# hieunghia-pat/OpenViIC

Measured on AMD Instinct MI355X. Metric: captions/sec (whole node) at beam=5, 50 regions x d2048, higher is better.
Workload: dtype f32; 1 GPU; standard_transformer beam=5, B=256 per GPU, 50x2048 synthetic regions, V=10201, max_len=20, random-init weights; global_batch=256, parallelism=dp1, streams=4

## Files before the change

### include/ovc.h

```cpp
#ifndef OVC_H_
#define OVC_H_

#include <stddef.h>
#include <stdint.h>

#ifdef __cplusplus
extern "C" {
#endif

typedef void* ovc_stream;

#define OVC_OK            0
#define OVC_EINVAL       -1
#define OVC_EWORKSPACE   -2
#define OVC_ELAUNCH      -3
#define OVC_EDEVICE      -4

#define OVC_MAX_LAYERS    8
#define OVC_MAX_LEVELS    4
#define OVC_MAX_BEAM      8
#define OVC_MAX_SEGMENTS  8
#define OVC_MAX_REGIONS   1024
#define OVC_MAX_LEN       256

// ... 302 lines not shown

int ovc_debug_force_gemm_tiling(int tiling);
int ovc_debug_clear_tuning(void);
int ovc_debug_linear_tiling(const float* x, int K, const float* W, const float* bias, float* y, int M, int N,
                            int tiling, int ksplit, int iters, ovc_stream stream);
int ovc_debug_attention_mem_backward(const float* q, const float* k, const float* v, const float* dout, const uint8_t* mask,
                                     const float* m_k, const float* m_v, int B, int n, int h, int dk, int m, float* P, float* dS,
                                     float* dq, float* dk_out, float* dv_out, float* part_k, float* part_v, float* colpart,
                                     float* d_mk, float* d_mv, ovc_stream stream);

size_t ovc_debug_vocab_select_bytes(int B, int width, int V, int k);
int ovc_debug_vocab_select(const float* x, const float* fc, const float* running, const float* alive, int B, int width,
                           int V, int d, int k, int transposed, int kchains, void* scratch, size_t scratch_bytes, int64_t* chosen,
                           float* score, ovc_stream stream);

size_t ovc_split_weight_bytes(int N, int K, int mode);
int ovc_split_weight(const float* W, int N, int K, int mode, void* planes, ovc_stream stream);
int ovc_debug_linear_planes(const float* x, int K, const float* W, const void* planes, const float* bias, float* y,
                            int M, int N, int tiling, int ksplit, int iters, ovc_stream stream);
int ovc_debug_repeat_linear(const float* x, int K, const float* W, const float* bias, float* y,
                            int M, int N, int iters, ovc_stream stream);

size_t ovc_debug_decode_self_partial_bytes(int t, int rows, int h, int d_k);
int ovc_debug_decode_self_attention(const float* q, int ldq, const float* kcache, const float* vcache, size_t pos_stride, int ldkv,
                                    const int32_t* anc, int anc_ld, const uint8_t* padflag, int pad_ld, int t, int width, int rows,
                                    int h, int d_k, float* out, int ldo, void* partials, size_t partial_bytes, const int32_t* gate,
                                    int per_row, ovc_stream stream);
int ovc_debug_decode_cross_attention(const float* q, int ldq, const float* kx, const float* vx, size_t level_stride, int ldkv,
                                     const uint8_t* encmask, int N, int width, int B, int heads, int d_k, int levels, float* out,
                                     size_t out_level_stride, int ldo, const int32_t* gate, ovc_stream stream);
int ovc_debug_decode_self_form(int t, int width, int rows, int h, int d_k, int per_row);
int ovc_debug_decode_cross_form(int N, int width, int h, int d_k);

typedef struct {
    const float* teacher_logp;
    float weight;
} ovc_distill;
size_t ovc_train_distill_workspace_bytes(const ovc_model* m, int B, int N, int T, int dropout);
int ovc_forward_backward_distill(const ovc_model* m, const ovc_model* grads, const float* features, const float* boxes, int B, int N,
                                 const int64_t* tokens, const int64_t* targets, int T, void* workspace, size_t workspace_bytes,
                                 float* loss_out, int use_graph, ovc_stream stream, const ovc_distill* distill,
                                 const ovc_dropout* dropout);
int ovc_ensemble_combine(const float* const* logps, int M, long rows, int V, int renormalise, float* out, ovc_stream stream);

#ifdef __cplusplus
}
#endif
#endif
```

### openviic_amd/csrc/attention.hip

```cpp
#include <cstdlib>
#include <mutex>

#include "common.h"

namespace {

constexpr int kQTile = 64;
constexpr int kLdQK = 68;

struct AttnArgs {
    const float* q; const float* k; const float* v; float* out;
    int b, nq, nk, h, dk, dv;
    const uint8_t* mask; long mask_sb, mask_sq;
    const float* geometry;
    const float* mem_k; const float* mem_v; int m; float mem_scale_k, mem_scale_v;
    int nkp;
    int qtiles;
};

__global__ __launch_bounds__(256) void attention_mfma_kernel(AttnArgs p) {
    extern __shared__ __attribute__((aligned(16))) float lds[];
    const int tid = threadIdx.x, lane = tid & 63, wave = tid >> 6;
    const int qt = blockIdx.x % p.qtiles;
    const int hd = (blockIdx.x / p.qtiles) % p.h;
// ... 474 lines not shown
                                      hipFuncAttributeMaxDynamicSharedMemorySize, 96 * 1024);                         \
        });                                                                                                           \
        hipLaunchKernelGGL((attention_tiled_kernel<KG, DVT>), grid, block, bytes, ovc_hip_stream(stream), p);         \
    } while (0)
        if (hmax <= 16) OVC_ATT_TILED(2, 1); else if (hmax <= 32) OVC_ATT_TILED(4, 1); else OVC_ATT_TILED(8, 2);
#undef OVC_ATT_TILED
        OVC_RETURN_IF_LAUNCH_FAILED();
        return OVC_OK;
    }
    const size_t lds_bytes = sizeof(float) * ((size_t)kQTile * kLdQK + 2 * (size_t)p.nkp * kLdQK + (size_t)kQTile * (p.nkp + 4));
    static std::once_flag attr_once;
    std::call_once(attr_once, [] {
        (void)hipFuncSetAttribute(reinterpret_cast<const void*>(attention_mfma_kernel),
                                  hipFuncAttributeMaxDynamicSharedMemorySize, 128 * 1024);
    });
    hipLaunchKernelGGL(attention_mfma_kernel, dim3(b * h * p.qtiles), dim3(256), lds_bytes, ovc_hip_stream(stream), p);
    OVC_RETURN_IF_LAUNCH_FAILED();
    return OVC_OK;
}


constexpr int kSelfMaxHeads = 32;

template <int CH, int KB = 1>
__global__ __launch_bounds__(256) void decode_self_attention_kernel(DecodeSelfArgs p) {
#include "bodies/decode_self_attention_kernel.inc"
}
template <int CH, int KB = 1>
__global__ __launch_bounds__(256) void decode_self_attention_kernel_gated(DecodeSelfArgs p, const int32_t* __restrict__ gate) {
    if (ovc_gate_closed(gate)) return;
#include "bodies/decode_self_attention_kernel.inc"
}

template <int NT, int SB, bool CHUNKED = false>
__global__ __launch_bounds__(256) void decode_self_attention_mfma_kernel(DecodeSelfArgs p) {
#include "bodies/decode_self_attention_mfma_kernel.inc"
}
template <int NT, int SB, bool CHUNKED = false>
__global__ __launch_bounds__(256) void decode_self_attention_mfma_kernel_gated(DecodeSelfArgs p, const int32_t* __restrict__ gate) {
    if (ovc_gate_closed(gate)) return;
#include "bodies/decode_self_attention_mfma_kernel.inc"
}

__global__ __launch_bounds__(256) void decode_self_merge_kernel(DecodeSelfArgs p, int rows, int chunks) {
#include "bodies/decode_self_merge_kernel.inc"
}
__global__ __launch_bounds__(256) void decode_self_merge_kernel_gated(DecodeSelfArgs p, int rows, int chunks, const int32_t* __restrict__ gate) {
    if (ovc_gate_closed(gate)) return;
#include "bodies/decode_self_merge_kernel.inc"
}

constexpr int kFormSelfMfma = 100, kFormSelfChunked = 200, kFormSelfRows = 300;
constexpr int kFormCrossMfma = 400, kFormCrossTiled = 500, kFormCrossLds = 600;

static int decode_self_form(int t, int W, int rows, int h, int dk, bool per_row) {
    if (t < 0 || t >= OVC_MAX_LEN || h <= 0 || h > kSelfMaxHeads) return OVC_EINVAL;
    if ((dk & (dk - 1)) || dk < 4 || dk > 64) return OVC_EINVAL;
    const int hk = h * dk;
    if (hk > 1024) return OVC_EINVAL;
    const bool per_image = !per_row && W >= 1 && W <= OVC_MAX_BEAM && rows % W == 0 && dk >= 16;
    const int SB = dk >> 4, CH = hk <= 256 ? 1 : hk <= 512 ? 2 : 4;
    if (t >= 64) {
        if (per_image) return kFormSelfChunked + (W <= 1 ? 1 : W <= 2 ? 2 : W <= 4 ? 4 : W <= 5 ? 5 : 8) * 10 + SB;
        return kFormSelfRows + CH * 10 + 4;
    }
    const int worst = t == 0 ? 1 : W * (t + 1);
    if (per_image && worst <= 112) {
        const int tiles = (worst + 15) / 16;
        return kFormSelfMfma + (tiles <= 1 ? 1 : tiles <= 2 ? 2 : tiles <= 4 ? 4 : 7) * 10 + SB;
    }
    return kFormSelfRows + CH * 10 + 1;
}

static int decode_self_attention_as(const DecodeSelfArgs& p, int rows, bool per_row, hipStream_t stream, const int32_t* gate) {
    if (p.dk != p.dv) return OVC_EINVAL;
    const int form = decode_self_form(p.t, p.width, rows, p.h, p.dk, per_row);
    if (form < 0) return form;
    const int W = p.width;
    const bool chunked = form >= kFormSelfChunked && form < kFormSelfRows;
    if (chunked && (!p.part_o || !p.part_ml)) return OVC_EINVAL;
    const int chunks = (p.t + kSelfChunk) / kSelfChunk;
    switch (form) {
#define OVC_SELF(NT, SB)                                                                                             \
    case kFormSelfMfma + NT * 10 + SB: {                                                                             \
        const dim3 grid(rows / W, (p.h + 3) / 4), block(256);                                                        \
        if (gate) hipLaunchKernelGGL((decode_self_attention_mfma_kernel_gated<NT, SB>), grid, block, 0, stream, p, gate); \
        else hipLaunchKernelGGL((decode_self_attention_mfma_kernel<NT, SB>), grid, block, 0, stream, p);            \
    } break
#define OVC_SELF_CHUNKED(NT, SB)                                                                                     \
    case kFormSelfChunked + NT * 10 + SB: {                                                                          \
        const dim3 grid(rows / W, (p.h + 3) / 4, chunks), block(256);                                                \
        if (gate) hipLaunchKernelGGL((decode_self_attention_mfma_kernel_gated<NT, SB, true>), grid, block, 0, stream, p, gate); \
        else hipLaunchKernelGGL((decode_self_attention_mfma_kernel<NT, SB, true>), grid, block, 0, stream, p);      \
    } break
#define OVC_SELF_ROWS(CH, KB)                                                                                        \
    case kFormSelfRows + CH * 10 + KB:                                                                               \
        if (gate) hipLaunchKernelGGL((decode_self_attention_kernel_gated<CH, KB>), dim3(rows), dim3(256), 0, stream, p, gate); \
        else hipLaunchKernelGGL((decode_self_attention_kernel<CH, KB>), dim3(rows), dim3(256), 0, stream, p);       \
        break
#define OVC_SELF_SB(M, NT) M(NT, 1); M(NT, 2); M(NT, 4)
        OVC_SELF_SB(OVC_SELF, 1); OVC_SELF_SB(OVC_SELF, 2); OVC_SELF_SB(OVC_SELF, 4); OVC_SELF_SB(OVC_SELF, 7);
        OVC_SELF_SB(OVC_SELF_CHUNKED, 1); OVC_SELF_SB(OVC_SELF_CHUNKED, 2); OVC_SELF_SB(OVC_SELF_CHUNKED, 4);
        OVC_SELF_SB(OVC_SELF_CHUNKED, 5); OVC_SELF_SB(OVC_SELF_CHUNKED, 8);
        OVC_SELF_ROWS(1, 1); OVC_SELF_ROWS(2, 1); OVC_SELF_ROWS(4, 1);
        OVC_SELF_ROWS(1, 4); OVC_SELF_ROWS(2, 4); OVC_SELF_ROWS(4, 4);
#undef OVC_SELF_SB
#undef OVC_SELF_ROWS
#undef OVC_SELF_CHUNKED
#undef OVC_SELF
        default: return OVC_EINVAL;
    }
    OVC_RETURN_IF_LAUNCH_FAILED();
    if (chunked) {
// ... 112 lines not shown

extern "C" size_t ovc_debug_decode_self_partial_bytes(int t, int rows, int h, int d_k) {
    if (t < 64 || t >= OVC_MAX_LEN || rows < 1 || !debug_heads_ok(h, d_k)) return 0;
    const size_t chunks = (size_t)(t + kSelfChunk) / kSelfChunk;
    return sizeof(float) * chunks * rows * ((size_t)h * d_k + 2 * (size_t)h);
}

extern "C" int ovc_debug_decode_self_attention(const float* q, int ldq, const float* kcache, const float* vcache, size_t pos_stride,
                                               int ldkv, const int32_t* anc, int anc_ld, const uint8_t* padflag, int pad_ld, int t,
                                               int width, int rows, int h, int d_k, float* out, int ldo, void* partials,
                                               size_t partial_bytes, const int32_t* gate, int per_row, ovc_stream stream) {
    if (!q || !kcache || !vcache || !padflag || !out || (t > 0 && !anc)) return OVC_EINVAL;
    if (!debug_self_shape_ok(t, width, rows, h, d_k)) return OVC_EINVAL;
    const int hk = h * d_k;
    if (ldq < hk || ldkv < hk || ldo < hk || (ldq & 3) || (ldkv & 3) || (ldo & 3) || (pos_stride & 3)) return OVC_EINVAL;
    if (anc_ld < t || pad_ld < rows) return OVC_EINVAL;
    if (!ovc_aligned16(q) || !ovc_aligned16(kcache) || !ovc_aligned16(vcache) || !ovc_aligned16(out)) return OVC_EINVAL;
    const size_t need = ovc_debug_decode_self_partial_bytes(t, rows, h, d_k);
    if (need && (!partials || !ovc_aligned16(partials) || partial_bytes < need)) return OVC_EINVAL;
    if (const int rc = ovc_device_guard()) return rc;
    DecodeSelfArgs p{};
    p.q = q; p.ldq = ldq; p.kcache = kcache; p.vcache = vcache; p.pos_stride = pos_stride; p.ldkv = ldkv;
    p.anc = anc; p.anc_ld = anc_ld; p.padflag = padflag; p.pad_ld = pad_ld;
    p.t = t; p.width = width; p.h = h; p.dk = d_k; p.dv = d_k;
    p.out = out; p.ldo = ldo;
    if (need) {
        const size_t chunks = (size_t)(t + kSelfChunk) / kSelfChunk;
        p.part_o = static_cast<float*>(partials);
        p.part_ml = p.part_o + chunks * rows * hk;
    }
    return decode_self_attention_as(p, rows, per_row != 0, ovc_hip_stream(stream), gate);
}

extern "C" int ovc_debug_decode_cross_attention(const float* q, int ldq, const float* kx, const float* vx, size_t level_stride, int ldkv,
                                                const uint8_t* encmask, int N, int width, int B, int heads, int d_k, int levels,
                                                float* out, size_t out_level_stride, int ldo, const int32_t* gate, ovc_stream stream) {
    if (!q || !kx || !vx || !out || B < 1 || levels < 1 || levels > OVC_MAX_LEVELS) return OVC_EINVAL;
    if (!debug_cross_shape_ok(N, width, heads, d_k)) return OVC_EINVAL;
    const int hk = heads * d_k;
    if (ldq < hk || ldkv < hk || ldo < hk || (ldq & 3) || (ldkv & 3) || (ldo & 3) || (level_stride & 3) || (out_level_stride & 3)) return OVC_EINVAL;
    if (!ovc_aligned16(q) || !ovc_aligned16(kx) || !ovc_aligned16(vx) || !ovc_aligned16(out)) return OVC_EINVAL;
    if (const int rc = ovc_device_guard()) return rc;
    DecodeCrossArgs p{};
    p.q = q; p.ldq = ldq; p.kx = kx; p.vx = vx; p.level_stride = level_stride; p.ldkv = ldkv;
    p.encmask = encmask; p.n = N; p.width = width; p.heads = heads; p.dk = d_k; p.dv = d_k;
    p.out = out; p.out_level_stride = out_level_stride; p.ldo = ldo;
    return ovc_decode_cross_attention(p, B, heads, levels, ovc_hip_stream(stream), gate);
}
```

### openviic_amd/csrc/bodies/decode_self_attention_mfma_kernel.inc

```
    constexpr int kPos = CHUNKED ? kSelfChunk : 64;
    __shared__ unsigned short keyinfo[NT * 16];
    __shared__ uint8_t keypad[NT * 16];
    __shared__ uint8_t sl[OVC_MAX_BEAM][kPos];
    __shared__ int nkeys_shared;
    const int lane = threadIdx.x & 63, wave = threadIdx.x >> 6;
    const int b = blockIdx.x, t = p.t, W = p.width;
    const int j0 = CHUNKED ? (int)blockIdx.z * kSelfChunk : 0;
    const int hd = min((int)blockIdx.y * 4 + wave, p.h - 1);
    const bool live = (int)blockIdx.y * 4 + wave < p.h;
    const int r = lane & 15, kq = lane >> 4;

    const float* qg = p.q + (size_t)(b * W + min(r, W - 1)) * p.ldq + hd * p.dk;
    f32x4 qf[SB];
#pragma unroll
    for (int S = 0; S < SB; ++S) qf[S] = *reinterpret_cast<const f32x4*>(qg + 16 * S + 4 * kq);

    if (wave == 0) {
        const int j = j0 + lane;
        const int wj = j == 0 ? 1 : W;
        int slot[OVC_MAX_BEAM];
        uint8_t pad[OVC_MAX_BEAM];
        unsigned mask = 0;
        if (j <= t && lane < kPos) {
#pragma unroll
            for (int i = 0; i < OVC_MAX_BEAM; ++i)
                slot[i] = i < W ? (j == t ? i : p.anc[(size_t)(b * W + i) * p.anc_ld + j] - b * wj) : 0;
#pragma unroll
            for (int l = 0; l < OVC_MAX_BEAM; ++l) pad[l] = l < wj ? p.padflag[(size_t)j * p.pad_ld + b * wj + l] : 0;
#pragma unroll
            for (int i = 0; i < OVC_MAX_BEAM; ++i)
                if (i < W) {
                    const int s = min(max(slot[i], 0), wj - 1);
                    sl[i][j - j0] = (uint8_t)s;
                    mask |= 1u << s;
                }
        }
        const int cnt = __popc(mask);
        int incl = cnt;
#pragma unroll
        for (int off = 1; off < 64; off <<= 1) {
            const int up = __shfl_up(incl, off, 64);
            if (lane >= off) incl += up;
        }
        int n = incl - cnt;
#pragma unroll
        for (int l = 0; l < OVC_MAX_BEAM; ++l)
            if (mask & (1u << l)) {
                if (n < NT * 16) { keyinfo[n] = (unsigned short)((j << 3) | l); keypad[n] = pad[l]; }
                ++n;
            }
        if (lane == 63) nkeys_shared = min(incl, NT * 16);
    }
    __syncthreads();
    const int nkeys = nkeys_shared;

    f32x4 kf[NT][SB];
#pragma unroll
    for (int T = 0; T < NT; ++T) {
        if (16 * T < nkeys) {
            const int info = keyinfo[min(16 * T + r, nkeys - 1)];
            const int j = info >> 3, l = info & 7;
            const float* krow = p.kcache + (size_t)j * p.pos_stride + (size_t)(b * (j == 0 ? 1 : W) + l) * p.ldkv + hd * p.dk + 4 * kq;
#pragma unroll
            for (int S = 0; S < SB; ++S) kf[T][S] = *reinterpret_cast<const f32x4*>(krow + 16 * S);
        }
    }
    if (r >= W) {
#pragma unroll
        for (int S = 0; S < SB; ++S) qf[S] = f32x4{0.f, 0.f, 0.f, 0.f};
    }
    f32x4 st[NT];
#pragma unroll
    for (int T = 0; T < NT; ++T) st[T] = f32x4{0.f, 0.f, 0.f, 0.f};
#pragma unroll
    for (int T = 0; T < NT; ++T) {
        if (16 * T < nkeys) {
#pragma unroll
            for (int S = 0; S < SB; ++S)
#pragma unroll
                for (int e = 0; e < 4; ++e) st[T] = __builtin_amdgcn_mfma_f32_16x16x4f32(kf[T][S][e], qf[S][e], st[T], 0, 0, 0);
        }
    }

    const int vc = 4 * min(r, (p.dv >> 2) - 1);
    f32x4 vf[NT][4];
#pragma unroll
    for (int T = 0; T < NT; ++T) {
        if (16 * T < nkeys) {
#pragma unroll
            for (int g = 0; g < 4; ++g) {
                const int info = keyinfo[min(16 * T + 4 * kq + g, nkeys - 1)];
                const int j = info >> 3, l = info & 7;
                vf[T][g] = *reinterpret_cast<const f32x4*>(p.vcache + (size_t)j * p.pos_stride +
                                                           (size_t)(b * (j == 0 ? 1 : W) + l) * p.ldkv + hd * p.dv + vc);
            }
        }
    }

    const float scale_div = sqrtf((float)p.dk);
    const int beam = min(r, W - 1);
    float mx = -INFINITY;
#pragma unroll
    for (int T = 0; T < NT; ++T) {
#pragma unroll
        for (int g = 0; g < 4; ++g) {
            const int key = 16 * T + 4 * kq + g;
            float s = -INFINITY;
            if (key < nkeys) {
                const int info = keyinfo[key];
                if (!keypad[key] && sl[beam][(info >> 3) - j0] == (info & 7)) s = st[T][g] / scale_div;
            }
            st[T][g] = s;
            mx = fmaxf(mx, s);
        }
    }
    mx = fmaxf(mx, __shfl_xor(mx, 16, 64));
    mx = fmaxf(mx, __shfl_xor(mx, 32, 64));
    const float mref = CHUNKED && mx == -INFINITY ? 0.f : mx;
    float sum = 0.f;
#pragma unroll
    for (int T = 0; T < NT; ++T)
#pragma unroll
        for (int g = 0; g < 4; ++g) {
            const float e = expf(st[T][g] - mref);
            st[T][g] = e;
            sum += e;
        }
    sum += __shfl_xor(sum, 16, 64);
    sum += __shfl_xor(sum, 32, 64);
    if constexpr (!CHUNKED) {
#pragma unroll
        for (int T = 0; T < NT; ++T)
#pragma unroll
            for (int g = 0; g < 4; ++g) st[T][g] = st[T][g] / sum;
    }

    f32x4 acc[4];
#pragma unroll
    for (int e = 0; e < 4; ++e) acc[e] = f32x4{0.f, 0.f, 0.f, 0.f};
#pragma unroll
    for (int T = 0; T < NT; ++T) {
        if (16 * T < nkeys) {
#pragma unroll
            for (int g = 0; g < 4; ++g)
#pragma unroll
                for (int e = 0; e < 4; ++e) acc[e] = __builtin_amdgcn_mfma_f32_16x16x4f32(vf[T][g][e], st[T][g], acc[e], 0, 0, 0);
        }
    }
    if (live && r < W) {
        float* orow;
        if constexpr (CHUNKED) {
            const size_t prow = (size_t)blockIdx.z * gridDim.x * W + b * W + r;
            orow = p.part_o + prow * p.h * p.dv + hd * p.dv;
            if (kq == 0) reinterpret_cast<float2*>(p.part_ml)[prow * p.h + hd] = make_float2(mx, sum);
        } else {
            orow = p.out + (size_t)(b * W + r) * p.ldo + hd * p.dv;
        }
#pragma unroll
        for (int g = 0; g < 4; ++g) {
            const int dvb = 16 * kq + 4 * g;
            if (dvb < p.dv) *reinterpret_cast<f32x4*>(orow + dvb) = f32x4{acc[0][g], acc[1][g], acc[2][g], acc[3][g]};
        }
    }
```

### openviic_amd/csrc/common.h

```cpp
#pragma once
#include <hip/hip_runtime.h>
#include <stdint.h>
#include "../../include/ovc.h"

#define OVC_WAVE 64

#define OVC_RETURN_IF_LAUNCH_FAILED()                      \
    do {                                                   \
        if (hipGetLastError() != hipSuccess) return OVC_ELAUNCH; \
    } while (0)

typedef float f32x2 __attribute__((ext_vector_type(2)));
typedef float f32x4 __attribute__((ext_vector_type(4)));
typedef float f32x16 __attribute__((ext_vector_type(16)));

static inline hipStream_t ovc_hip_stream(ovc_stream s) { return reinterpret_cast<hipStream_t>(s); }

int ovc_device_guard();

static inline bool ovc_aligned16(const void* p) { return (reinterpret_cast<uintptr_t>(p) & 15u) == 0; }

#ifdef OVC_MEASUREMENT_HOOKS
#include <cstdlib>
#define OVC_HOOK_ENV(name) getenv(name)
// ... 102 lines not shown
    int drop_cols = 0;
};

int ovc_gemm_launch(const GemmArgs& args, hipStream_t stream, const GemmLaunchOpts& opts = GemmLaunchOpts{});
int ovc_gemm_pick_tiling(const GemmArgs& args, const GemmLaunchOpts& opts = GemmLaunchOpts{});
int ovc_gemm_tiling_class(int tiling);
constexpr int kMaxKSplit = 4;
int ovc_layer_norm_parts(const float* parts, int nparts, long part_stride, const float* bias, const float* residual,
                         const float* gamma, const float* beta, const uint8_t* zero_rows, float eps, float* y,
                         int rows, int d, hipStream_t stream, const int32_t* gate = nullptr);
int ovc_layer_norm_gated(const float* x, const float* residual, const float* gamma, const float* beta, const float* add, int add_rows,
                         const uint8_t* zero_rows, float eps, float* y, int rows, int d, hipStream_t stream, const int32_t* gate);
int ovc_sigmoid_gate_gated(const float* a, const float* g, float* y, long n, hipStream_t stream, const int32_t* gate);
const char* ovc_gemm_tiling_name(int tiling);

struct DecodeSelfArgs {
    const float* q;
    int ldq;
    const float* kcache;
    const float* vcache;
    size_t pos_stride;
    int ldkv;
    const int32_t* anc;
    int anc_ld;
    const uint8_t* padflag;
    int pad_ld;
    int t;
    int width;
    int h, dk, dv;
    float* out;
    int ldo;
    float* part_o;
    float* part_ml;
};
constexpr int kSelfChunk = 16;
int ovc_decode_self_attention(const DecodeSelfArgs& p, int rows, hipStream_t stream, const int32_t* gate = nullptr);

struct DecodeCrossArgs {
    const float* q;
    int ldq;
    const float* kx;
    const float* vx;
    size_t level_stride;
    int ldkv;
    const uint8_t* encmask;
    int n, width;
    int heads, dk, dv;
    float* out;
    size_t out_level_stride;
    int ldo;
};
int ovc_decode_cross_attention(const DecodeCrossArgs& p, int B, int h, int levels, hipStream_t stream, const int32_t* gate = nullptr);

struct BeamSelectArgs {
    const float* logits;
    int ld;
    int is_logp;
    const float* running;
    const float* alive;
    int width, V, k;
    float* cand_v;
    int* cand_i;
    int64_t* chosen;
    float* score;
    float* masked_logp;
    float* row_max_out;
    float* row_lsum_out;
// ... 99 lines not shown
```

### openviic_amd/csrc/engine.hip

```cpp
#include <algorithm>
#include <array>
#include <cstdlib>
#include <list>
#include <map>
#include <memory>
#include <atomic>
#include <cmath>
#include <mutex>
#include <tuple>
#include <vector>

#include "common.h"
#include "backward.h"
#include "dropout.h"

namespace {

#define TRY(expr)                          \
    do {                                   \
        const int _rc = (expr);            \
        if (_rc != OVC_OK) return _rc;     \
    } while (0)
#define RUN(expr)                          \
    do {                                   \
// ... 38 lines not shown
        }
        (void)hipEventDestroy(r.start); (void)hipEventDestroy(r.stop);
    }
    g_profile.clear();
}

struct Bump {
    char* base; size_t off;
    template <typename T> T* take(size_t count) {
        off = (off + 255) & ~(size_t)255;
        T* p = base ? reinterpret_cast<T*>(base + off) : nullptr;
        off += count * sizeof(T);
        return p;
    }
};

struct EncTape { float *q, *k, *v, *att, *ya, *x1, *ff, *yf, *out; };
struct DecTape { float *q, *k, *v, *att, *ys, *x1, *qc, *attc, *yc, *x2, *ff, *yf, *out; };
struct ClTape { float *k[2], *v[2], *att, *ya, *o2p, *a1, *h2; };
struct Tape { EncTape enc[OVC_MAX_LAYERS]; DecTape dec[OVC_MAX_LAYERS]; ClTape cl; };

struct Workspace {
    const Tape* tape;
    uint8_t* enc_mask; float* pe; float* xe[2]; float* eq; float* ek; float* ev; float* eatt; float* ey;
    float* eff; float* einfo; float* egate; float* geometry; float* enc_levels;
    float* kx; float* vx;
    float* cl_out; float* cl_cat; float* cl_q;
    float* x; float* x1; float* x2; float* y; float* q; float* att; float* ff; float* info; float* gate;
    float* enc_att; float* alpha; float* mixed; float* ymesh;
    float* part;
    float* kc; float* vc;
    uint8_t* padflag;
    float* sa_part_o; float* sa_part_ml;
    float* logits;
    float* stats;
    float* running[2]; float* alive[2]; int32_t* hist[2]; float* lp[2]; int32_t* anc[2];
    int32_t* tok; float* cand_v; int32_t* cand_i; float* row_max; float* row_lsum; int32_t* order;
    float* all_buf;
    int64_t* out_ids; float* out_logp;
    int32_t* alive_count;
    int64_t* drop_seed; int32_t* steps_dev;
    float* choice_rows; int32_t* choice_word; int32_t* choice_kept;
    uint8_t* self_mask; int32_t* tgt; float* tgt_logit; float* lse;
    Workspace* peers;
    size_t bytes;
};

int enc_heads(const ovc_model* m) { return m->enc_heads ? m->enc_heads : m->heads; }
int enc_dk(const ovc_model* m) { return m->enc_d_k ? m->enc_d_k : m->d_k; }
int enc_dv(const ovc_model* m) { return m->enc_d_v ? m->enc_d_v : m->d_v; }

bool heads_ok(int h, int dk, int dv) {
    if (dk != dv || dk < 4 || dk > 64 || (dk & (dk - 1))) return false;
    if (h <= 0 || h > 32 || h * dk > 1024) return false;
    return (h * dk) % 64 == 0;
}

bool model_ok(const ovc_model* m) {
    if (!m || m->abi != ovc_abi_version()) return false;
    if (m->n_enc < 1 || m->n_enc > OVC_MAX_LAYERS || m->n_dec < 1 || m->n_dec > OVC_MAX_LAYERS) return false;
    if (m->n_levels < 1 || m->n_levels > OVC_MAX_LEVELS) return false;
    if (m->d_model <= 0 || (m->d_model & 3) || m->d_model > 2048) return false;
    if (!heads_ok(m->heads, m->d_k, m->d_v)) return false;
    if ((m->d_feat & 3) || (m->d_ff & 3) || m->vocab <= 1) return false;
    if (m->d_feat <= 0 || m->d_ff <= 0 || m->memory < 0) return false;
    if (m->max_len < 1 || m->max_len > OVC_MAX_LEN) return false;
// ... 629 lines not shown
    for (int i = 0; i < c.ens_M; ++i) {
        const ovc_model* e = c.ens[i];
        if (!search_ok(e, alone) || e->precision != 0 || (e->vocab + 31) / 32 > kFusedVocabBlocks) return false;
        if (e->vocab != m->vocab || e->max_len != m->max_len || e->bos_idx != m->bos_idx || e->eos_idx != m->eos_idx ||
            e->pad_idx != m->pad_idx || e->d_feat != m->d_feat)
            return false;
    }
    return true;
}

bool search_ok(const ovc_model* m, const SearchCall& c) {
    if (!search_model_ok(m, c) || c.B <= 0 || c.N <= 0 || c.N > OVC_MAX_REGIONS || c.k <= 0 || c.k > OVC_MAX_BEAM) return false;
    if (c.sample && (m->precision != 0 || (m->vocab + 31) / 32 > kFusedVocabBlocks || c.plan ||
                     (c.form != SearchForm::Plain && c.form != SearchForm::Graph)))
        return false;
    if (c.has_options && (!c.sample || !ovc_sample_options_ok(c.temperature, c.top_k, c.top_p))) return false;
    if (c.constrained() && (m->precision != 0 || (m->vocab + 31) / 32 > kFusedVocabBlocks || c.sample || c.plan ||
                            (c.form != SearchForm::Plain && c.form != SearchForm::Graph) ||
                            !ovc_beam_constraints_ok(c.cons, m->vocab, m->max_len, c.k, m->eos_idx, m->pad_idx)))
        return false;
    if (c.ens_M != 0 && !ensemble_ok(m, c)) return false;
    return c.out_size > 0 && c.out_size <= c.k && (!c.plan || dropout_train_ok(m, c.B, c.N, m->max_len));
}

Workspace carve_search(const ovc_model* m, void* base, const SearchCall& c) {
    Workspace w = carve(m, base, c.B, c.N, c.k, c.all_logp_out != nullptr, c.plan != nullptr || c.sample);
    if (c.has_options) {
        Bump a{reinterpret_cast<char*>(base), w.bytes};
        const size_t R = (size_t)c.B * c.k;
        w.choice_rows = a.take<float>(R * (size_t)m->vocab);
        w.choice_word = a.take<int32_t>(R); w.choice_kept = a.take<int32_t>(R);
        w.bytes = (a.off + 255) & ~(size_t)255;
    }
    return w;
}

size_t carve_ensemble(const SearchCall& c, void* base, Workspace* ws) {
    size_t off = 0;
    for (int i = 0; i < c.ens_M; ++i) {
        ws[i] = carve_search(c.ens[i], base ? reinterpret_cast<char*>(base) + off : nullptr, c);
        off += ws[i].bytes;
        ws[i].peers = ws;
        if (i == 0) continue;
        const Workspace& s = ws[0];
        for (int j = 0; j < 2; ++j) {
            ws[i].running[j] = s.running[j]; ws[i].alive[j] = s.alive[j]; ws[i].hist[j] = s.hist[j]; ws[i].lp[j] = s.lp[j]; ws[i].anc[j] = s.anc[j];
        }
        ws[i].tok = s.tok; ws[i].padflag = s.padflag; ws[i].order = s.order; ws[i].out_ids = s.out_ids; ws[i].out_logp = s.out_logp;
        ws[i].all_buf = s.all_buf;
    }
    return off;
}

struct DecoderPass {
    enum Kind { Step, Sequence } kind;
    int rows;
    int B, N;
    const uint8_t* zero_rows;
    float* part;
    bool name_sites;
    int t, width, R; const int32_t* anc;
    int S, T;
    int site(int l, int j) const { return name_sites ? dec_site(l, j) : -1; }
};

int run_decoder_layer(Engine& e, Workspace& w, int l, const DecoderPass& p, const DecTape& b, const float* x) {
    const ovc_model* m = e.m;
    const ovc_dec_layer& dl = m->dec[l];
    hipStream_t s = e.stream;
    const int d = m->d_model, hk = m->heads * m->d_k, hv = m->heads * m->d_v, lv = m->n_levels;
    const int rows = p.rows, B = p.B, N = p.N;
    const float scale = sqrtf((float)m->d_k);
    GemmArgs a{};
    a.A1 = x; a.lda1 = d; a.K1 = d; a.M = rows; a.seg_n = hk; a.nseg = 3; a.ldc = hk;
    a.seg[0] = e.seg(dl.self_att.q, b.q);
    a.seg[1] = e.seg(dl.self_att.k, b.k);
    a.seg[2] = e.seg(dl.self_att.v, b.v);
    TRY(e.gemm(a));
    if (p.kind == DecoderPass::Step) {
        DecodeSelfArgs sa{};
        sa.q = b.q; sa.ldq = hk; sa.pos_stride = (size_t)p.R * hk; sa.ldkv = hk;
        sa.kcache = b.k - p.t * sa.pos_stride; sa.vcache = b.v - p.t * sa.pos_stride;
        sa.anc = p.anc; sa.anc_ld = m->max_len; sa.padflag = w.padflag; sa.pad_ld = p.R; sa.t = p.t; sa.width = p.width;
        sa.h = m->heads; sa.dk = m->d_k; sa.dv = m->d_v; sa.out = b.att; sa.ldo = hv;
        sa.part_o = w.sa_part_o; sa.part_ml = w.sa_part_ml;
        if (!(debug_skip() & 2)) RUN(ovc_decode_self_attention(sa, rows, s, e.gate));
    } else {
        const int smem = dl.self_att.m_k ? m->memory : 0;
        RUN(ovc_attention(b.q, b.k, b.v, B * p.S, p.T, p.T, m->heads, m->d_k, m->d_v, w.self_mask, (long)p.T * p.T, p.T, nullptr,
                          dl.self_att.m_k, dl.self_att.m_v, smem, scale, sqrtf((float)(smem > 0 ? smem : 1)), b.att, s));
    }
    TRY(e.linear_ln(b.att, hv, dl.self_att.o, x, dl.self_att.ln, nullptr, b.ys, p.part, b.x1, rows, p.site(l, 0)));
    TRY(e.aoa(dl.self_att, x, b.x1, w.info, w.gate, rows));

    TRY(e.linear(b.x1, d, dl.cross_att.q, nullptr, b.qc, rows, hk, 0));
    if (p.kind == DecoderPass::Step) {
        DecodeCrossArgs ca{};
        ca.q = b.qc; ca.ldq = hk;
        ca.kx = w.kx + (size_t)l * lv * B * N * hk; ca.vx = w.vx + (size_t)l * lv * B * N * hv;
        ca.level_stride = (size_t)B * N * hk; ca.ldkv = hk; ca.encmask = w.enc_mask; ca.n = N; ca.width = p.width;
        ca.heads = m->heads; ca.dk = m->d_k; ca.dv = m->d_v; ca.out = b.attc; ca.out_level_stride = (size_t)rows * hv; ca.ldo = hv;
        if (!(debug_skip() & 4)) RUN(ovc_decode_cross_attention(ca, B, m->heads, lv, s, e.gate));
    } else {
        const int cmem = dl.cross_att.m_k ? m->memory : 0;
        for (int lvl = 0; lvl < lv; ++lvl) {
            const size_t off = ((size_t)l * lv + lvl) * B * N * hk;
            RUN(ovc_attention(b.qc, w.kx + off, w.vx + off, B, p.S * p.T, N, m->heads, m->d_k, m->d_v, w.enc_mask, N, 0, nullptr,
                              dl.cross_att.m_k, dl.cross_att.m_v, cmem, scale, sqrtf((float)(cmem > 0 ? cmem : 1)),
                              b.attc + (size_t)lvl * rows * hv, s));
        }
    }
    const float* ffn_in;
    if (m->dec_kind == OVC_DEC_MESHED) {
        const size_t nrd = (size_t)rows * d;
        if (!dl.cross_att.aoa_i.w) {
            GemmArgs o{};
            o.A1 = b.attc; o.lda1 = hv; o.K1 = hv; o.M = lv * rows; o.seg_n = d; o.nseg = 1; o.ldc = d;
            o.R = b.x1; o.ldr = d; o.res_mod = rows;
// ... 1735 lines not shown
```

### openviic_amd/native.py

```python
import ctypes
import os
from ctypes import POINTER, c_char_p, c_double, c_float, c_int, c_int32, c_int64, c_long, c_size_t, c_void_p

OVC_MAX_LAYERS = 8
OVC_MAX_LEVELS = 4
OVC_MAX_BEAM = 8
OVC_MAX_REGIONS = 1024
OVC_MAX_LEN = 256
OVC_MAX_BANNED = 16
OVC_MAX_ENSEMBLE = 4
OVC_PROFILE_CLASSES = 4
ABI_VERSION = 8

_ERRORS = {-1: "OVC_EINVAL (bad argument / unsupported shape)", -2: "OVC_EWORKSPACE (workspace too small)",
           -3: "OVC_ELAUNCH (HIP launch failed)",
           -4: "OVC_EDEVICE (the library is bound to another device: one device per process)"}


class OvcError(RuntimeError):
    pass


class Lin(ctypes.Structure):
    _fields_ = [("w", c_void_p), ("b", c_void_p), ("planes", c_void_p)]
# ... 175 lines not shown
                                            POINTER(c_int32), c_int, c_void_p, c_size_t, c_void_p, c_void_p, c_void_p, c_void_p]),
    "ovc_beam_search_constrained_graph": (c_int, [POINTER(Model), c_void_p, c_void_p, c_int, c_int, c_int, c_int, c_int, c_int,
                                                  POINTER(c_int32), c_int, c_void_p, c_size_t, c_void_p, c_void_p, c_void_p]),
    "ovc_debug_beam_constrained_update_bytes": (c_size_t, [c_int, c_int, c_int, c_int, c_int]),
    "ovc_debug_beam_constrained_update": (c_int, [c_void_p, c_void_p, c_void_p, c_void_p, c_int, c_int, c_int, c_int, c_int, c_int,
                                                  c_int, c_int, c_int, POINTER(c_int32), c_int, c_void_p, c_size_t, c_void_p,
                                                  c_void_p, c_void_p, c_void_p, c_void_p, c_void_p]),
    "ovc_ensemble_ok": (c_int, [POINTER(POINTER(Model)), c_int, c_int, c_int, c_int]),
    "ovc_ensemble_workspace_bytes": (c_size_t, [POINTER(POINTER(Model)), c_int, c_int, c_int, c_int, c_int]),
    "ovc_ensemble_beam_search": (c_int, [POINTER(POINTER(Model)), c_int, c_void_p, c_void_p, c_int, c_int, c_int, c_int, c_void_p, c_size_t,
                                         c_void_p, c_void_p, c_void_p, c_void_p]),
    "ovc_ensemble_beam_search_graph": (c_int, [POINTER(POINTER(Model)), c_int, c_void_p, c_void_p, c_int, c_int, c_int, c_int, c_void_p,
                                               c_size_t, c_void_p, c_void_p, c_void_p]),
    "ovc_debug_ensemble_update_bytes": (c_size_t, [c_int, c_int, c_int, c_int, c_int]),
    "ovc_debug_ensemble_update": (c_int, [c_void_p, c_void_p, c_void_p, c_int, c_int, c_int, c_int, c_int, c_int, c_int, c_void_p, c_size_t,
                                          c_void_p, c_void_p, c_void_p, c_void_p, c_void_p, c_void_p, c_void_p, c_void_p]),
    "ovc_cider_reward": (c_int, [POINTER(Cider), c_void_p, c_void_p, c_int, c_int, c_int, c_void_p, c_void_p]),
    "ovc_adam_chunk_count": (c_long, [c_void_p, c_int]),
    "ovc_adam_chunk_fill": (c_long, [c_void_p, c_int, c_void_p, c_long]),
    "ovc_adam_step": (c_int, [c_void_p, c_int, c_void_p, c_long, c_double, c_double, c_double, c_double, c_long, c_void_p, c_void_p]),
    "ovc_grad_norm": (c_int, [c_void_p, c_int, c_void_p, c_long, c_double, c_void_p, c_void_p, c_void_p]),
    "ovc_scst_advantage_bytes": (c_size_t, [c_int, c_int, c_int]),
    "ovc_scst_advantage": (c_int, [c_void_p, c_void_p, c_int, c_int, c_int, c_void_p, c_void_p, c_void_p, c_size_t, c_void_p]),
    "ovc_caption_metrics_bytes": (c_size_t, [c_int, c_int, c_int]),
    "ovc_caption_metrics": (c_int, [POINTER(EvalCorpus), c_void_p, c_void_p, c_int, c_int, c_void_p, c_void_p, c_size_t, c_void_p]),
    "ovc_debug_decode_self_partial_bytes": (c_size_t, [c_int, c_int, c_int, c_int]),
    "ovc_debug_decode_self_attention": (c_int, [c_void_p, c_int, c_void_p, c_void_p, c_size_t, c_int, c_void_p, c_int, c_void_p, c_int,
                                                c_int, c_int, c_int, c_int, c_int, c_void_p, c_int, c_void_p, c_size_t, c_void_p,
                                                c_int, c_void_p]),
    "ovc_debug_decode_cross_attention": (c_int, [c_void_p, c_int, c_void_p, c_void_p, c_size_t, c_int, c_void_p, c_int, c_int, c_int,
                                                 c_int, c_int, c_int, c_void_p, c_size_t, c_int, c_void_p, c_void_p]),
    "ovc_debug_decode_self_form": (c_int, [c_int, c_int, c_int, c_int, c_int, c_int]),
    "ovc_debug_decode_cross_form": (c_int, [c_int, c_int, c_int, c_int]),
    "ovc_graph_cache_clear": (c_int, []),
    "ovc_profile_enable": (c_int, [c_int]),
    "ovc_profile_read": (c_int, [c_int, c_int, POINTER(c_int64), POINTER(c_double), POINTER(c_double)]),
    "ovc_profile_overhead_ms": (c_double, []),
    "ovc_profile_kernel_name": (c_char_p, [c_int]),
}

APPENDED_ABI8 = ("ovc_dropout_mask_rows", "ovc_beam_search_dropout_workspace_bytes", "ovc_beam_search_dropout",
                 "ovc_train_beams_dropout_workspace_bytes", "ovc_sequence_backward_dropout",
                 "ovc_adam_chunk_count", "ovc_adam_chunk_fill", "ovc_adam_step", "ovc_debug_attention_mem_backward",
                 "ovc_scst_advantage_bytes", "ovc_scst_advantage", "ovc_caption_metrics_bytes", "ovc_caption_metrics",
                 "ovc_grad_norm", "ovc_train_smoothed_workspace_bytes", "ovc_forward_backward_smoothed",
                 "ovc_sample_workspace_bytes", "ovc_sample", "ovc_sample_graph",
                 "ovc_sample_shaped_workspace_bytes", "ovc_sample_shaped", "ovc_sample_shaped_graph",
                 "ovc_sample_choice_workspace_bytes", "ovc_sample_choice",
                 "ovc_debug_decode_self_partial_bytes", "ovc_debug_decode_self_attention", "ovc_debug_decode_cross_attention",
                 "ovc_debug_decode_self_form", "ovc_debug_decode_cross_form",
                 "ovc_search_constraints_ok", "ovc_beam_search_constrained", "ovc_beam_search_constrained_graph",
                 "ovc_debug_beam_constrained_update_bytes", "ovc_debug_beam_constrained_update",
                 "ovc_ensemble_ok", "ovc_ensemble_workspace_bytes", "ovc_ensemble_beam_search", "ovc_ensemble_beam_search_graph",
                 "ovc_debug_ensemble_update_bytes", "ovc_debug_ensemble_update",
                 "ovc_train_distill_workspace_bytes", "ovc_forward_backward_distill", "ovc_ensemble_combine")

_lib = None


def load():
    global _lib
    if _lib is not None:
        return _lib
    if not os.path.exists(LIBRARY_PATH):
        raise OvcError("HIP library not built: {} is missing -- run `python -m openviic_amd.csrc.build` "
                       "(there is no CPU fallback)".format(LIBRARY_PATH))
    lib = ctypes.CDLL(LIBRARY_PATH)
    for name, (restype, argtypes) in SIGNATURES.items():
        fn = getattr(lib, name, None)
        if fn is None:
            if os.environ.get("OVC_LIBRARY") and name in APPENDED_ABI8:
                continue
            raise AttributeError("{} does not export {}".format(LIBRARY_PATH, name))
        fn.restype, fn.argtypes = restype, argtypes
    if lib.ovc_abi_version() != ABI_VERSION:
        raise OvcError("libovc.so ABI {} != binding ABI {}; rebuild".format(lib.ovc_abi_version(), ABI_VERSION))
    _lib = lib
    return lib


def check(status: int, what: str) -> None:
    if status != 0:
        raise OvcError("{} failed: {}".format(what, _ERRORS.get(status, status)))
# ... 6 lines not shown
```

Before: 21580 captions/s.

## Share decoder self-attention key list across layers via global record

The MFMA decode self-attention kernel rebuilds, in every decoder layer, the per-image key list (beam slot map, key info, pad flags) from the ancestry and padflag arrays. Layer 0 now publishes that LDS record to a per-image global buffer, and later layers load it with one dword per thread, skipping the ancestry and pad gathers. It also adds a compile-time option to issue V loads before the score computation, which is off by default. The cost is an extra workspace buffer, a global write in layer 0, and extra validation and branching in the kernel.

```diff
diff --git a/include/ovc.h b/include/ovc.h
--- a/include/ovc.h
+++ b/include/ovc.h
@@ -358,6 +358,13 @@
 int ovc_debug_decode_self_form(int t, int width, int rows, int h, int d_k, int per_row);
 int ovc_debug_decode_cross_form(int N, int width, int h, int d_k);
 
+#define OVC_SELF_LIST_BYTES 1024
+#define OVC_SELF_LIST_KEYS 112
+size_t ovc_debug_decode_self_list_bytes(int B);
+int ovc_debug_decode_self_list(const float* q, int ldq, const float* kcache, const float* vcache, size_t pos_stride, int ldkv,
+                               const int32_t* anc, int anc_ld, const uint8_t* padflag, int pad_ld, int t, int width, int rows,
+                               int h, int d_k, float* out, int ldo, void* list, size_t list_bytes, int mode, ovc_stream stream);
+
 typedef struct {
     const float* teacher_logp;
     float weight;
diff --git a/openviic_amd/csrc/attention.hip b/openviic_amd/csrc/attention.hip
--- a/openviic_amd/csrc/attention.hip
+++ b/openviic_amd/csrc/attention.hip
@@ -530,6 +530,11 @@
 #include "bodies/decode_self_attention_kernel.inc"
 }
 
+#ifndef OVC_SELF_V_EARLY_MAX_NT
+#define OVC_SELF_V_EARLY_MAX_NT 0
+#endif
+constexpr bool ovc_self_v_early(int NT, int SB) { return NT <= OVC_SELF_V_EARLY_MAX_NT; }
+
 template <int NT, int SB, bool CHUNKED = false>
 __global__ __launch_bounds__(256) void decode_self_attention_mfma_kernel(DecodeSelfArgs p) {
 #include "bodies/decode_self_attention_mfma_kernel.inc"
@@ -577,6 +582,8 @@
     const int W = p.width;
     const bool chunked = form >= kFormSelfChunked && form < kFormSelfRows;
     if (chunked && (!p.part_o || !p.part_ml)) return OVC_EINVAL;
+    if (p.list_mode < kSelfListBuild || p.list_mode > kSelfListConsume) return OVC_EINVAL;
+    if (form < kFormSelfChunked && p.list_mode != kSelfListBuild && !p.list) return OVC_EINVAL;
     const int chunks = (p.t + kSelfChunk) / kSelfChunk;
     switch (form) {
 #define OVC_SELF(NT, SB)                                                                                             \
@@ -755,6 +762,31 @@
     return decode_self_attention_as(p, rows, per_row != 0, ovc_hip_stream(stream), gate);
 }
 
+extern "C" size_t ovc_debug_decode_self_list_bytes(int B) { return B >= 1 ? (size_t)B * OVC_SELF_LIST_BYTES : 0; }
+
+extern "C" int ovc_debug_decode_self_list(const float* q, int ldq, const float* kcache, const float* vcache, size_t pos_stride, int ldkv,
+                                          const int32_t* anc, int anc_ld, const uint8_t* padflag, int pad_ld, int t, int width, int rows,
+                                          int h, int d_k, float* out, int ldo, void* list, size_t list_bytes, int mode, ovc_stream stream) {
+    if (!q || !kcache || !vcache || !padflag || !out || !list || (t > 0 && !anc)) return OVC_EINVAL;
+    if (mode != kSelfListPublish && mode != kSelfListConsume) return OVC_EINVAL;
+    if (!debug_self_shape_ok(t, width, rows, h, d_k)) return OVC_EINVAL;
+    const int form = decode_self_form(t, width, rows, h, d_k, false);
+    if (form < kFormSelfMfma || form >= kFormSelfChunked) return OVC_EINVAL;
+    const int hk = h * d_k;
+    if (ldq < hk || ldkv < hk || ldo < hk || (ldq & 3) || (ldkv & 3) || (ldo & 3) || (pos_stride & 3)) return OVC_EINVAL;
+    if (anc_ld < t || pad_ld < rows) return OVC_EINVAL;
+    if (!ovc_aligned16(q) || !ovc_aligned16(kcache) || !ovc_aligned16(vcache) || !ovc_aligned16(out) || !ovc_aligned16(list)) return OVC_EINVAL;
+    if (list_bytes < ovc_debug_decode_self_list_bytes(rows / width)) return OVC_EINVAL;
+    if (const int rc = ovc_device_guard()) return rc;
+    DecodeSelfArgs p{};
+    p.q = q; p.ldq = ldq; p.kcache = kcache; p.vcache = vcache; p.pos_stride = pos_stride; p.ldkv = ldkv;
+    p.anc = anc; p.anc_ld = anc_ld; p.padflag = padflag; p.pad_ld = pad_ld;
+    p.t = t; p.width = width; p.h = h; p.dk = d_k; p.dv = d_k;
+    p.out = out; p.ldo = ldo;
+    p.list_mode = mode; p.list = static_cast<uint32_t*>(list);
+    return decode_self_attention_as(p, rows, false, ovc_hip_stream(stream), nullptr);
+}
+
 extern "C" int ovc_debug_decode_cross_attention(const float* q, int ldq, const float* kx, const float* vx, size_t level_stride, int ldkv,
                                                 const uint8_t* encmask, int N, int width, int B, int heads, int d_k, int levels,
                                                 float* out, size_t out_level_stride, int ldo, const int32_t* gate, ovc_stream stream) {
diff --git a/openviic_amd/csrc/bodies/decode_self_attention_mfma_kernel.inc b/openviic_amd/csrc/bodies/decode_self_attention_mfma_kernel.inc
--- a/openviic_amd/csrc/bodies/decode_self_attention_mfma_kernel.inc
+++ b/openviic_amd/csrc/bodies/decode_self_attention_mfma_kernel.inc
@@ -1,36 +1,60 @@
     constexpr int kPos = CHUNKED ? kSelfChunk : 64;
-    __shared__ unsigned short keyinfo[NT * 16];
-    __shared__ uint8_t keypad[NT * 16];
-    __shared__ uint8_t sl[OVC_MAX_BEAM][kPos];
-    __shared__ int nkeys_shared;
+    constexpr int kKeys = CHUNKED ? NT * 16 : kSelfListKeys;
+    constexpr int kOffInfo = OVC_MAX_BEAM * kPos, kOffPad = kOffInfo + 2 * kKeys, kOffN = kOffPad + kKeys;
+    constexpr int kListBytes = CHUNKED ? kOffN + 4 : OVC_SELF_LIST_BYTES;
+    static_assert(kOffN % 4 == 0 && kOffN + 4 <= kListBytes && kListBytes % 4 == 0, "key list layout");
+    static_assert(CHUNKED || (NT * 16 <= kSelfListKeys && OVC_SELF_LIST_BYTES == 4 * 256), "a record is one dword per thread of the workgroup");
+    __shared__ __attribute__((aligned(16))) uint32_t listw[kListBytes / 4];
+    uint8_t (*sl)[kPos] = reinterpret_cast<uint8_t (*)[kPos]>(listw);
+    unsigned short* keyinfo = reinterpret_cast<unsigned short*>(reinterpret_cast<uint8_t*>(listw) + kOffInfo);
+    uint8_t* keypad = reinterpret_cast<uint8_t*>(listw) + kOffPad;
+    int& nkeys_shared = *reinterpret_cast<int*>(reinterpret_cast<uint8_t*>(listw) + kOffN);
     const int lane = threadIdx.x & 63, wave = threadIdx.x >> 6;
     const int b = blockIdx.x, t = p.t, W = p.width;
     const int j0 = CHUNKED ? (int)blockIdx.z * kSelfChunk : 0;
     const int hd = min((int)blockIdx.y * 4 + wave, p.h - 1);
     const bool live = (int)blockIdx.y * 4 + wave < p.h;
     const int r = lane & 15, kq = lane >> 4;
+    const bool consume = !CHUNKED && p.list_mode == kSelfListConsume;
+
+    uint32_t rec = 0;
+    if (consume) rec = p.list[(size_t)b * (OVC_SELF_LIST_BYTES / 4) + threadIdx.x];
 
     const float* qg = p.q + (size_t)(b * W + min(r, W - 1)) * p.ldq + hd * p.dk;
     f32x4 qf[SB];
 #pragma unroll
     for (int S = 0; S < SB; ++S) qf[S] = *reinterpret_cast<const f32x4*>(qg + 16 * S + 4 * kq);
 
-    if (wave == 0) {
+    if (consume) {
+        if constexpr (!CHUNKED) listw[threadIdx.x] = rec;
+    } else if (wave == 0) {
         const int j = j0 + lane;
         const int wj = j == 0 ? 1 : W;
-        int slot[OVC_MAX_BEAM];
+        const bool listed = j <= t && lane < kPos;
+        int anc_raw[OVC_MAX_BEAM];
+        uint8_t pad_raw[OVC_MAX_BEAM];
+#pragma unroll
+        for (int i = 0; i < OVC_MAX_BEAM; ++i) { anc_raw[i] = 0; pad_raw[i] = 0; }
+        if (listed) {
+            if (t > 0) {
+                const int32_t* arow = p.anc + (size_t)(b * W) * p.anc_ld + min(j, t - 1);
+#pragma unroll
+                for (int i = 0; i < OVC_MAX_BEAM; ++i) anc_raw[i] = arow[(size_t)min(i, W - 1) * p.anc_ld];
+            }
+            const uint8_t* prow = p.padflag + (size_t)j * p.pad_ld + b * wj;
+#pragma unroll
+            for (int l = 0; l < OVC_MAX_BEAM; ++l) pad_raw[l] = prow[min(l, wj - 1)];
+        }
         uint8_t pad[OVC_MAX_BEAM];
         unsigned mask = 0;
-        if (j <= t && lane < kPos) {
 #pragma unroll
-            for (int i = 0; i < OVC_MAX_BEAM; ++i)
-                slot[i] = i < W ? (j == t ? i : p.anc[(size_t)(b * W + i) * p.anc_ld + j] - b * wj) : 0;
-#pragma unroll
-            for (int l = 0; l < OVC_MAX_BEAM; ++l) pad[l] = l < wj ? p.padflag[(size_t)j * p.pad_ld + b * wj + l] : 0;
+        for (int l = 0; l < OVC_MAX_BEAM; ++l) pad[l] = l < wj ? pad_raw[l] : 0;
+        if (listed) {
 #pragma unroll
             for (int i = 0; i < OVC_MAX_BEAM; ++i)
                 if (i < W) {
-                    const int s = min(max(slot[i], 0), wj - 1);
+                    const int slot = j == t ? i : anc_raw[i] - b * wj;
+                    const int s = min(max(slot, 0), wj - 1);
                     sl[i][j - j0] = (uint8_t)s;
                     mask |= 1u << s;
                 }
@@ -65,6 +89,24 @@
             for (int S = 0; S < SB; ++S) kf[T][S] = *reinterpret_cast<const f32x4*>(krow + 16 * S);
         }
     }
+    constexpr bool kVEarly = !CHUNKED && ovc_self_v_early(NT, SB);
+    const int vc = 4 * min(r, (p.dv >> 2) - 1);
+    f32x4 vf[NT][4];
+    auto load_v = [&]() {
+#pragma unroll
+        for (int T = 0; T < NT; ++T) {
+            if (16 * T < nkeys) {
+#pragma unroll
+                for (int g = 0; g < 4; ++g) {
+                    const int info = keyinfo[min(16 * T + 4 * kq + g, nkeys - 1)];
+                    const int j = info >> 3, l = info & 7;
+                    vf[T][g] = *reinterpret_cast<const f32x4*>(p.vcache + (size_t)j * p.pos_stride +
+                                                               (size_t)(b * (j == 0 ? 1 : W) + l) * p.ldkv + hd * p.dv + vc);
+                }
+            }
+        }
+    };
+    if constexpr (kVEarly) load_v();
     if (r >= W) {
 #pragma unroll
         for (int S = 0; S < SB; ++S) qf[S] = f32x4{0.f, 0.f, 0.f, 0.f};
@@ -82,20 +124,7 @@
         }
     }
 
-    const int vc = 4 * min(r, (p.dv >> 2) - 1);
-    f32x4 vf[NT][4];
-#pragma unroll
-    for (int T = 0; T < NT; ++T) {
-        if (16 * T < nkeys) {
-#pragma unroll
-            for (int g = 0; g < 4; ++g) {
-                const int info = keyinfo[min(16 * T + 4 * kq + g, nkeys - 1)];
-                const int j = info >> 3, l = info & 7;
-                vf[T][g] = *reinterpret_cast<const f32x4*>(p.vcache + (size_t)j * p.pos_stride +
-                                                           (size_t)(b * (j == 0 ? 1 : W) + l) * p.ldkv + hd * p.dv + vc);
-            }
-        }
-    }
+    if constexpr (!kVEarly) load_v();
 
     const float scale_div = sqrtf((float)p.dk);
     const int beam = min(r, W - 1);
@@ -162,3 +191,6 @@
             if (dvb < p.dv) *reinterpret_cast<f32x4*>(orow + dvb) = f32x4{acc[0][g], acc[1][g], acc[2][g], acc[3][g]};
         }
     }
+    if constexpr (!CHUNKED) {
+        if (p.list_mode == kSelfListPublish && blockIdx.y == 0) p.list[(size_t)b * (OVC_SELF_LIST_BYTES / 4) + threadIdx.x] = listw[threadIdx.x];
+    }
diff --git a/openviic_amd/csrc/common.h b/openviic_amd/csrc/common.h
--- a/openviic_amd/csrc/common.h
+++ b/openviic_amd/csrc/common.h
@@ -158,7 +158,11 @@
     int ldo;
     float* part_o;
     float* part_ml;
-};
+    int list_mode;
+    uint32_t* list;
+};
+constexpr int kSelfListBuild = 0, kSelfListPublish = 1, kSelfListConsume = 2;
+constexpr int kSelfListKeys = OVC_SELF_LIST_KEYS;
 constexpr int kSelfChunk = 16;
 int ovc_decode_self_attention(const DecodeSelfArgs& p, int rows, hipStream_t stream, const int32_t* gate = nullptr);
 
diff --git a/openviic_amd/csrc/engine.hip b/openviic_amd/csrc/engine.hip
--- a/openviic_amd/csrc/engine.hip
+++ b/openviic_amd/csrc/engine.hip
@@ -94,6 +94,7 @@
     float* kc; float* vc;
     uint8_t* padflag;
     float* sa_part_o; float* sa_part_ml;
+    uint32_t* sa_list;
     float* logits;
     float* stats;
     float* running[2]; float* alive[2]; int32_t* hist[2]; float* lp[2]; int32_t* anc[2];
@@ -789,6 +790,11 @@
         w.choice_word = a.take<int32_t>(R); w.choice_kept = a.take<int32_t>(R);
         w.bytes = (a.off + 255) & ~(size_t)255;
     }
+    if (m->n_dec > 1) {
+        Bump a{reinterpret_cast<char*>(base), w.bytes};
+        w.sa_list = a.take<uint32_t>((size_t)c.B * (OVC_SELF_LIST_BYTES / 4));
+        w.bytes = (a.off + 255) & ~(size_t)255;
+    }
     return w;
 }
 
@@ -841,6 +847,7 @@
         sa.anc = p.anc; sa.anc_ld = m->max_len; sa.padflag = w.padflag; sa.pad_ld = p.R; sa.t = p.t; sa.width = p.width;
         sa.h = m->heads; sa.dk = m->d_k; sa.dv = m->d_v; sa.out = b.att; sa.ldo = hv;
         sa.part_o = w.sa_part_o; sa.part_ml = w.sa_part_ml;
+        if (w.sa_list && m->n_dec > 1) { sa.list = w.sa_list; sa.list_mode = l == 0 ? kSelfListPublish : kSelfListConsume; }
         if (!(debug_skip() & 2)) RUN(ovc_decode_self_attention(sa, rows, s, e.gate));
     } else {
         const int smem = dl.self_att.m_k ? m->memory : 0;
diff --git a/openviic_amd/native.py b/openviic_amd/native.py
--- a/openviic_amd/native.py
+++ b/openviic_amd/native.py
@@ -231,6 +231,9 @@
                                                  c_int, c_int, c_int, c_void_p, c_size_t, c_int, c_void_p, c_void_p]),
     "ovc_debug_decode_self_form": (c_int, [c_int, c_int, c_int, c_int, c_int, c_int]),
     "ovc_debug_decode_cross_form": (c_int, [c_int, c_int, c_int, c_int]),
+    "ovc_debug_decode_self_list_bytes": (c_size_t, [c_int]),
+    "ovc_debug_decode_self_list": (c_int, [c_void_p, c_int, c_void_p, c_void_p, c_size_t, c_int, c_void_p, c_int, c_void_p, c_int,
+                                           c_int, c_int, c_int, c_int, c_int, c_void_p, c_int, c_void_p, c_size_t, c_int, c_void_p]),
     "ovc_graph_cache_clear": (c_int, []),
     "ovc_profile_enable": (c_int, [c_int]),
     "ovc_profile_read": (c_int, [c_int, c_int, POINTER(c_int64), POINTER(c_double), POINTER(c_double)]),
@@ -248,6 +251,7 @@
                  "ovc_sample_choice_workspace_bytes", "ovc_sample_choice",
                  "ovc_debug_decode_self_partial_bytes", "ovc_debug_decode_self_attention", "ovc_debug_decode_cross_attention",
                  "ovc_debug_decode_self_form", "ovc_debug_decode_cross_form",
+                 "ovc_debug_decode_self_list_bytes", "ovc_debug_decode_self_list",
                  "ovc_search_constraints_ok", "ovc_beam_search_constrained", "ovc_beam_search_constrained_graph",
                  "ovc_debug_beam_constrained_update_bytes", "ovc_debug_beam_constrained_update",
                  "ovc_ensemble_ok", "ovc_ensemble_workspace_bytes", "ovc_ensemble_beam_search", "ovc_ensemble_beam_search_graph",
```

Measured after the change: 21750 captions/s (median of 6 runs). Within noise of the previous version (+0.8%).
